# NSagan271/dietgpu_fork

Measured on AMD Instinct MI355X. Metric: encode+decode GB/s (+ratio) on bf16 batch at 1/2/4/8 MI355X vs HBM roofline, higher is better.
Workload: dtype u32; 1 GPU; c2: batch=256 x 1 MiB bf16 N(0,1) per GPU; batch_per_gpu=256, words_per_tensor=524288, prob_bits=10, api=floatCompress + floatDecompress (pointer API, C ABI), parallelism=dp1 (independent shards + RCCL size all-gather)

## Files before the change

### dietgpu_fork_amd/csrc/decode.h

```cpp
#pragma once

#include <type_traits>

#include "archive.h"

namespace dietgpu {

namespace dec {
constexpr int kThreads = 256;
constexpr int kWaves = kThreads / 64;
constexpr uint32_t kRing = 512;
constexpr uint32_t kRefill = 256;
constexpr uint32_t kWPL = kRefill / 64;
constexpr uint32_t kSegSteps = 8;
constexpr uint32_t kSegWords = kSegSteps * 32;
constexpr uint32_t kUnroll = 4;
constexpr uint32_t kChunk = kSegWords / 32;
}

template <int FT>
struct DecCfg {
  static constexpr int S = FloatTraits<FT>::kSegs;
  static constexpr int kBlocksPerWave = 2;
  static constexpr int kBlocksPerWG = dec::kWaves * kBlocksPerWave;
  static constexpr uint32_t kHalfStreams = dec::kWaves * S * 2;
  static constexpr uint32_t kRingBytes = kHalfStreams * dec::kRing * 2;
  static constexpr uint32_t kSegBytes = kHalfStreams * dec::kSegWords * 2;
  __host__ __device__ static constexpr uint32_t lutBytes(int pb) { return S * (8u << pb); }
  __host__ __device__ static constexpr uint32_t ldsBytes(int pb) {
    return lutBytes(pb) + kRingBytes + kSegBytes;
  }
};

struct DStream {
  uint32_t x;
  lp<uint16_t> ring;
  lp<const uint16_t> ringLane;
  int32_t ptr[2];
  int32_t lo[2];
  gp<const uint16_t> data[2];
  u32x2 pf[2];
};

__device__ __forceinline__ u32x2 ld4w(gp<const uint16_t> p, bool vec) {
  if (vec) return *(gp<const u32x2>)p;
  return u32x2{uint32_t(p[0]) | (uint32_t(p[1]) << 16), uint32_t(p[2]) | (uint32_t(p[3]) << 16)};
}

__device__ __forceinline__ void ringPrefetch(DStream& p, int hh, uint32_t lane, bool vec) {
  const int32_t nlo = max(0, p.lo[hh] - int32_t(dec::kRefill));
  if (p.lo[hh] > 0 && int32_t(dec::kWPL * lane) < p.lo[hh] - nlo)
    p.pf[hh] = ld4w(p.data[hh] + nlo + dec::kWPL * lane, vec);
}

__device__ __forceinline__ void ringEnsure(DStream& p, uint32_t lane, bool vec) {
#pragma unroll
  for (int hh = 0; hh < 2; ++hh) {
    if (p.lo[hh] > 0 && p.ptr[hh] - int32_t(32 * dec::kUnroll) < p.lo[hh]) {
      const int32_t nlo = max(0, p.lo[hh] - int32_t(dec::kRefill));
      if (int32_t(dec::kWPL * lane) < p.lo[hh] - nlo)
        *(lp<u32x2>)(p.ring + hh * dec::kRing + ((nlo + dec::kWPL * lane) & (dec::kRing - 1))) = p.pf[hh];
      p.lo[hh] = nlo;
      ringPrefetch(p, hh, lane, vec);
    }
  }
}

template <bool kMask, int NC>
__device__ __forceinline__ void decStepAll(DStream* const (&p)[NC], const bool (&valid)[NC],
                                           lp<const u32x2> const (&lut)[NC], uint32_t mask, int pb,
                                           uint32_t hv, uint32_t (&e0)[NC]) {
  u32x2 e[NC];
#pragma unroll
  for (int c = 0; c < NC; ++c) e[c] = lut[c][p[c]->x & mask];
  __builtin_amdgcn_sched_barrier(0);
  uint32_t xn[NC], v[NC];
  bool rd[NC];
#pragma unroll
  for (int c = 0; c < NC; ++c) {
    DStream& q = *p[c];
    xn[c] = __umul24(e[c].x, q.x >> pb) + e[c].y;
    if (kMask) xn[c] = valid[c] ? xn[c] : q.x;
    rd[c] = kMask ? (valid[c] && xn[c] < kMinState) : (xn[c] < kMinState);
    const uint64_t vote = ballot(rd[c]);
    const int32_t cLo = __popc(uint32_t(vote));
    const int32_t cHi = __popc(uint32_t(vote >> 32));
    const int32_t baseLo = q.ptr[0] - cLo;
    const int32_t diff = q.ptr[1] - q.ptr[0] - cHi;
    q.ptr[0] = baseLo;
    q.ptr[1] -= cHi;
    const uint32_t vbase = uint32_t(baseLo) + (hv & uint32_t(diff));
    const uint32_t idx = __builtin_amdgcn_mbcnt_hi(uint32_t(vote >> 32),
                                                   __builtin_amdgcn_mbcnt_lo(uint32_t(vote), vbase));
    v[c] = q.ringLane[idx & (dec::kRing - 1)];
    e0[c] = e[c].x;
  }
  __builtin_amdgcn_sched_barrier(0);
#pragma unroll
  for (int c = 0; c < NC; ++c)
    p[c]->x = __builtin_amdgcn_perm(xn[c], v[c], rd[c] ? 0x05040100u : 0x07060504u);
}

template <bool kMask, int S>
__device__ __forceinline__ void decSteps(DStream* const (&chains)[S], lp<const u32x2> const (&lut)[S],
                                         uint32_t mask, int pb, uint32_t hv, lp<uint16_t> const (&segLane)[S],
                                         int tr0, int32_t tBot, uint32_t l, uint32_t uw) {
#pragma unroll
  for (int u = int(dec::kUnroll) - 1; u >= 0; --u) {
    const int tr = tr0 + u;
    bool vld[S];
#pragma unroll
    for (int s = 0; s < S; ++s) vld[s] = !kMask || uint32_t(tBot + tr) * 32 + l < uw;
    uint32_t e0[S];
    decStepAll<kMask, S>(chains, vld, lut, mask, pb, hv, e0);
#pragma unroll
    for (int s = 0; s < S; ++s)
      if (vld[s]) segLane[s][tr * 32] = uint16_t(e0[s] >> 16);
  }
}

__device__ __forceinline__ uint32_t upperHalfMask(uint32_t lane) {
  uint32_t hv = lane >= 32 ? ~0u : 0u;
  asm volatile("" : "+v"(hv));
  return hv;
}

__device__ __forceinline__ void bindStream(DStream& d, lp<uint16_t>& segLane, lp<uint16_t> ringAll,
                                           lp<uint16_t> segAll, uint32_t hs, uint32_t hv, uint32_t l) {
  d.ring = ringAll + hs * 2 * dec::kRing;
  d.ringLane = d.ring + (hv & dec::kRing);
  segLane = segAll + hs * 2 * dec::kSegWords + (hv & dec::kSegWords) + l;
}

__device__ __forceinline__ void openHalf(DStream& d, int hh, gp<const uint16_t> data, uint2 e, bool has,
                                         uint32_t lane, bool vecIn) {
  d.ptr[hh] = 0;
  d.lo[hh] = 0;
  d.data[hh] = data;
  d.pf[hh] = u32x2{0, 0};
  if (has) {
    const uint32_t ex = readfirst(e.x), ey = readfirst(e.y);
    const int32_t cw = int32_t(ex & 0xffffu);
    d.ptr[hh] = cw;
    d.data[hh] = data + ey;
    const int32_t lo = cw > int32_t(dec::kRing) ? int32_t(roundUp(uint32_t(cw) - dec::kRing, dec::kWPL)) : 0;
    d.lo[hh] = lo;
#pragma unroll
    for (int q = 0; q < int(dec::kRing / dec::kRefill); ++q) {
      const int32_t a = lo + q * int32_t(dec::kRefill) + int32_t(dec::kWPL * lane);
      if (a < cw) *(lp<u32x2>)(d.ring + hh * dec::kRing + (a & (dec::kRing - 1))) = ld4w(d.data[hh] + a, vecIn);
    }
    ringPrefetch(d, hh, lane, vecIn);
  }
}

__device__ __forceinline__ void setPrioRemaining(uint32_t left, uint32_t total) {
  const uint32_t q = total ? min(3u, (4u * left) / total) : 0u;
  if (q == 3) __builtin_amdgcn_s_setprio(3);
  else if (q == 2) __builtin_amdgcn_s_setprio(2);
  else if (q == 1) __builtin_amdgcn_s_setprio(1);
  else __builtin_amdgcn_s_setprio(0);
}

template <int FT, int ACC = 0>
struct Join {
  static_assert(ACC == 0 || (FT != 0 && (ACC == 1 || (ACC == 2 && (FT == 1 || FT == 2)))),
                "accumulate: float archives only; an fp32 accumulator only for fp16 / bf16");
  using WordT = typename FloatTraits<FT>::WordT;
  using AccT = std::conditional_t<ACC == 2, uint32_t, WordT>;
  static constexpr int kR = FT == 0 ? 1 : (FT <= 2 ? 2 : (FT == 3 ? 6 : 12));
  static constexpr int kW = 2 * int(sizeof(WordT));
  static constexpr int kD = ACC == 0 ? 1 : 2 * int(sizeof(AccT));

  static __device__ __forceinline__ void load(uint32_t (&r)[kR], gp<const uint8_t> raw, uint32_t n,
                                              uint32_t i0) {
    if constexpr (FT == 1 || FT == 2) {
      const uint2 a = ld8(raw + i0);
      r[0] = a.x; r[1] = a.y;
    } else if constexpr (FT == 3) {
      const uint4 a = ld16(raw + 2 * i0);
      const uint2 h = ld8(raw + floatPlane2Offset(FT, n) + i0);
      r[0] = a.x; r[1] = a.y; r[2] = a.z; r[3] = a.w; r[4] = h.x; r[5] = h.y;
    } else if constexpr (FT == 4) {
      const uint4 a = ld16(raw + 4 * i0), b = ld16(raw + 4 * i0 + 16);
      const uint4 h = ld16(raw + floatPlane2Offset(FT, n) + 2 * i0);
      r[0] = a.x; r[1] = a.y; r[2] = a.z; r[3] = a.w;
      r[4] = b.x; r[5] = b.y; r[6] = b.z; r[7] = b.w;
      r[8] = h.x; r[9] = h.y; r[10] = h.z; r[11] = h.w;
    }
  }

  static __device__ __forceinline__ WordT one(uint32_t s0, uint32_t s1, gp<const uint8_t> raw,
                                              uint32_t n, uint32_t i) {
    if constexpr (FT == 0) {
      return WordT(s0);
    } else if constexpr (FT == 1) {
      return WordT((s0 << 8) | raw[i]);
    } else if constexpr (FT == 2) {
      const uint32_t r = raw[i];
      return WordT((s0 << 7) | (r >> 1) | ((r & 1u) << 15));
    } else if constexpr (FT == 3) {
      const uint32_t lo = ((gp<const uint16_t>)raw)[i];
      const uint32_t hb = raw[floatPlane2Offset(FT, n) + i];
      return rotr32((s0 << 24) | (hb << 16) | lo, 1);
    } else {
      const uint64_t lo = ((gp<const uint32_t>)raw)[i];
      const uint64_t hb = ((gp<const uint16_t>)(raw + floatPlane2Offset(FT, n)))[i];
      const uint64_t v = (uint64_t(s0) << 56) | (uint64_t(s1) << 48) | (hb << 32) | lo;
      return (v >> 1) | (v << 63);
    }
  }

  static __device__ __forceinline__ uint32_t pair16(uint32_t sp, uint32_t rw, int odd) {
    return __builtin_amdgcn_perm(sp, rw, odd ? 0x07030502u : 0x07010500u);
  }

  template <bool nt>
  static __device__ __forceinline__ void vec(gp<uint8_t> outB, uint32_t i0, const uint32_t (&s)[4],
                                             const uint32_t (&s1)[4], const uint32_t (&r)[kR]) {
    if constexpr (FT == 0) {
      const uint2 v = make_uint2(__builtin_amdgcn_perm(s[1], s[0], 0x07050301u),
                                 __builtin_amdgcn_perm(s[3], s[2], 0x07050301u));
      if constexpr (nt) st8nt(outB + i0, v);
      else st8(outB + i0, v);
    } else if constexpr (FT == 1 || FT == 2) {
      uint32_t o[4];
#pragma unroll
      for (int k = 0; k < 4; ++k) {
        const uint32_t t = pair16(s[k], r[k >> 1], k & 1);
        o[k] = FT == 1 ? t : (((t >> 1) & 0x7fff7fffu) | ((t << 15) & 0x80008000u));
      }
      if constexpr (nt) st16nt(outB + 2 * i0, make_uint4(o[0], o[1], o[2], o[3]));
      else st16(outB + 2 * i0, make_uint4(o[0], o[1], o[2], o[3]));
    } else if constexpr (FT == 3) {
      uint32_t o[8];
#pragma unroll
      for (int k = 0; k < 4; ++k) {
        const uint32_t h = pair16(s[k], r[4 + (k >> 1)], k & 1);
        const uint32_t w0 = __builtin_amdgcn_perm(h, r[k], 0x05040100u);
        const uint32_t w1 = __builtin_amdgcn_perm(h, r[k], 0x07060302u);
        o[2 * k] = __builtin_amdgcn_alignbit(w0, w0, 1);
        o[2 * k + 1] = __builtin_amdgcn_alignbit(w1, w1, 1);
      }
      gp<uint4> d = (gp<uint4>)(outB + 4 * i0);
      if constexpr (nt) {
        st16nt(d, make_uint4(o[0], o[1], o[2], o[3]));
        st16nt(d + 1, make_uint4(o[4], o[5], o[6], o[7]));
      } else {
        st16(d, make_uint4(o[0], o[1], o[2], o[3]));
        st16(d + 1, make_uint4(o[4], o[5], o[6], o[7]));
      }
    } else {
      gp<uint4> d = (gp<uint4>)(outB + 8 * i0);
#pragma unroll
      for (int k = 0; k < 4; ++k) {
        const uint32_t p = __builtin_amdgcn_perm(s[k], s1[k], 0x07030501u);
        const uint32_t vh0 = __builtin_amdgcn_perm(p, r[8 + k], 0x05040100u);
        const uint32_t vh1 = __builtin_amdgcn_perm(p, r[8 + k], 0x07060302u);
        const uint32_t l0 = r[2 * k], l1 = r[2 * k + 1];
        st16(d + k, make_uint4(__builtin_amdgcn_alignbit(vh0, l0, 1), __builtin_amdgcn_alignbit(l0, vh0, 1),
                               __builtin_amdgcn_alignbit(vh1, l1, 1), __builtin_amdgcn_alignbit(l1, vh1, 1)));
      }
    }
  }

  static __device__ __forceinline__ float widen(uint32_t h) {
    if constexpr (FT == 1) return float(__builtin_bit_cast(_Float16, uint16_t(h)));
    else return __builtin_bit_cast(float, h << 16);
  }
  static __device__ __forceinline__ uint32_t bf16Of(float f) {
    return __builtin_bit_cast(uint16_t, static_cast<__bf16>(f));
  }
  static __device__ __forceinline__ uint32_t f32Sum(uint32_t a, float x) {
    return __builtin_bit_cast(uint32_t, __builtin_bit_cast(float, a) + x);
  }
  static __device__ __forceinline__ uint32_t sumPk16(uint32_t a, uint32_t x) {
    if constexpr (FT == 1) {
      typedef _Float16 h2 __attribute__((ext_vector_type(2)));
      return __builtin_bit_cast(uint32_t, __builtin_bit_cast(h2, a) + __builtin_bit_cast(h2, x));
    } else {
      const float lo = __builtin_bit_cast(float, a << 16) + __builtin_bit_cast(float, x << 16);
      const float hi = __builtin_bit_cast(float, a & 0xffff0000u) + __builtin_bit_cast(float, x & 0xffff0000u);
      return bf16Of(lo) | (bf16Of(hi) << 16);
    }
  }
  static __device__ __forceinline__ AccT sumOne(AccT a, WordT x) {
    if constexpr (ACC == 2) {
      return f32Sum(a, widen(x));
    } else if constexpr (FT == 1) {
      return __builtin_bit_cast(uint16_t, _Float16(__builtin_bit_cast(_Float16, a) + __builtin_bit_cast(_Float16, x)));
    } else if constexpr (FT == 2) {
      return AccT(bf16Of(widen(a) + widen(x)));
    } else if constexpr (FT == 3) {
      return f32Sum(a, __builtin_bit_cast(float, x));
    } else {
      return __builtin_bit_cast(uint64_t, __builtin_bit_cast(double, a) + __builtin_bit_cast(double, x));
    }
  }

  static __device__ __forceinline__ void words(uint32_t (&o)[kW], const uint32_t (&s)[4], const uint32_t (&s1)[4],
                                               const uint32_t (&r)[kR]) {
    if constexpr (FT == 0) {
      o[0] = __builtin_amdgcn_perm(s[1], s[0], 0x07050301u);
      o[1] = __builtin_amdgcn_perm(s[3], s[2], 0x07050301u);
    } else if constexpr (FT == 1 || FT == 2) {
#pragma unroll
      for (int k = 0; k < 4; ++k) {
        const uint32_t t = pair16(s[k], r[k >> 1], k & 1);
        o[k] = FT == 1 ? t : (((t >> 1) & 0x7fff7fffu) | ((t << 15) & 0x80008000u));
      }
    } else if constexpr (FT == 3) {
#pragma unroll
      for (int k = 0; k < 4; ++k) {
        const uint32_t h = pair16(s[k], r[4 + (k >> 1)], k & 1);
        const uint32_t w0 = __builtin_amdgcn_perm(h, r[k], 0x05040100u);
        const uint32_t w1 = __builtin_amdgcn_perm(h, r[k], 0x07060302u);
        o[2 * k] = __builtin_amdgcn_alignbit(w0, w0, 1);
        o[2 * k + 1] = __builtin_amdgcn_alignbit(w1, w1, 1);
      }
    } else {
#pragma unroll
      for (int k = 0; k < 4; ++k) {
        const uint32_t p = __builtin_amdgcn_perm(s[k], s1[k], 0x07030501u);
        const uint32_t vh0 = __builtin_amdgcn_perm(p, r[8 + k], 0x05040100u);
        const uint32_t vh1 = __builtin_amdgcn_perm(p, r[8 + k], 0x07060302u);
        const uint32_t l0 = r[2 * k], l1 = r[2 * k + 1];
        o[4 * k] = __builtin_amdgcn_alignbit(vh0, l0, 1);
        o[4 * k + 1] = __builtin_amdgcn_alignbit(l0, vh0, 1);
        o[4 * k + 2] = __builtin_amdgcn_alignbit(vh1, l1, 1);
        o[4 * k + 3] = __builtin_amdgcn_alignbit(l1, vh1, 1);
      }
    }
  }

  static __device__ __forceinline__ void loadAcc(uint32_t (&d)[kD], gp<const uint8_t> accB, uint32_t i0) {
    gp<const u32x4> p = (gp<const u32x4>)(accB + uint64_t(sizeof(AccT)) * i0);
#pragma unroll
    for (int j = 0; j < kD / 4; ++j) {
      const u32x4 v = p[j];
      d[4 * j] = v.x; d[4 * j + 1] = v.y; d[4 * j + 2] = v.z; d[4 * j + 3] = v.w;
    }
  }

  static __device__ __forceinline__ void vecAcc(gp<uint8_t> accB, uint32_t i0, const uint32_t (&s)[4],
                                                const uint32_t (&s1)[4], const uint32_t (&r)[kR],
                                                const uint32_t (&d)[kD]) {
    gp<u32x4> p = (gp<u32x4>)(accB + uint64_t(sizeof(AccT)) * i0);
    uint32_t o[kW], t[kD];
    if constexpr (FT == 4) {
      loadAcc(t, accB, i0);
      words(o, s, s1, r);
#pragma unroll
      for (int k = 0; k < 8; ++k) {
        const uint64_t sum = sumOne(uint64_t(t[2 * k]) | (uint64_t(t[2 * k + 1]) << 32),
                                    uint64_t(o[2 * k]) | (uint64_t(o[2 * k + 1]) << 32));
        t[2 * k] = uint32_t(sum);
        t[2 * k + 1] = uint32_t(sum >> 32);
      }
    } else {
      words(o, s, s1, r);
      if constexpr (ACC == 2) {
#pragma unroll
        for (int k = 0; k < 4; ++k) {
          t[2 * k] = f32Sum(d[2 * k], widen(o[k]));
          t[2 * k + 1] = f32Sum(d[2 * k + 1], widen(o[k] >> 16));
        }
      } else if constexpr (FT == 3) {
#pragma unroll
        for (int k = 0; k < 8; ++k) t[k] = f32Sum(d[k], __builtin_bit_cast(float, o[k]));
      } else {
#pragma unroll
        for (int k = 0; k < 4; ++k) t[k] = sumPk16(d[k], o[k]);
      }
    }
#pragma unroll
    for (int j = 0; j < kD / 4; ++j) p[j] = u32x4{t[4 * j], t[4 * j + 1], t[4 * j + 2], t[4 * j + 3]};
  }
};

template <int S>
__device__ __forceinline__ void loadChunkSyms(lp<const uint16_t> q0, lp<const uint16_t> q1, uint32_t (&sv)[4],
                                              uint32_t (&sv1)[4]) {
  const u32x4 a0 = *(lp<const u32x4>)q0;
  sv[0] = a0.x; sv[1] = a0.y; sv[2] = a0.z; sv[3] = a0.w;
  if constexpr (S == 2) {
    const u32x4 b0 = *(lp<const u32x4>)q1;
    sv1[0] = b0.x; sv1[1] = b0.y; sv1[2] = b0.z; sv1[3] = b0.w;
  } else {
#pragma unroll
    for (int k = 0; k < 4; ++k) sv1[k] = 0;
  }
}

__device__ __forceinline__ bool clipChunk(uint32_t i0, uint32_t cnt, uint32_t rlo, uint32_t rhi, uint32_t& k0,
                                          uint32_t& k1) {
  k0 = i0 < rlo ? min(cnt, rlo - i0) : 0u;
  k1 = rhi > i0 ? min(cnt, rhi - i0) : 0u;
  return k0 < k1;
}

template <class J>
__device__ __forceinline__ void joinWords(gp<typename J::WordT> o, lp<const uint16_t> q0, lp<const uint16_t> q1,
                                          gp<const uint8_t> raw, uint32_t n, uint32_t i0, uint32_t k0, uint32_t k1) {
  for (uint32_t k = k0; k < k1; ++k) o[i0 + k] = J::one(q0[k] >> 8, q1[k] >> 8, raw, n, i0 + k);
}

template <int FT>
__device__ __forceinline__ uint32_t openArchive(gp<const uint8_t> base, int pb, bool& ok,
                                                gp<const uint8_t> (&arch)[DecCfg<FT>::S]) {
  constexpr int S = DecCfg<FT>::S;
  gp<const uint32_t> fh = (gp<const uint32_t>)base;
  uint32_t n;
  if constexpr (FT == 0) {
    n = fh[kAnsSize];
    ok = fh[kAnsMagic] == kANSMagicVersion;
  } else {
    n = fh[kFloatSize];
    ok = fh[kFloatMagic] == kFloatMagicVersion && (fh[kFloatType] & kTypeMask) == uint32_t(FT);
  }
  arch[0] = ansArchiveOf<FT>(base, n);
  if constexpr (S == 2) arch[S - 1] = arch[0] + fh[kFloatSecondAns];
#pragma unroll
  for (int s = 0; s < S; ++s) {
    gp<const uint32_t> ah = (gp<const uint32_t>)arch[s];
    ok = ok && ah[kAnsMagic] == kANSMagicVersion && (ah[kAnsPrecision] & kTypeMask) == uint32_t(pb) &&
         ah[kAnsSize] == n;
  }
  return n;
}

__device__ __forceinline__ void buildLut64(gp<const uint16_t> pdfIn, lp<u32x2> lut, int pb,
                                           uint32_t* scratch) {
  static_assert(dec::kThreads == kNumSymbols, "one symbol per thread");
  uint32_t* cdfS = scratch;
  uint32_t* pdfS = scratch + kNumSymbols;
  uint32_t* red = scratch + 2 * kNumSymbols;
  const uint32_t tid = threadIdx.x;
  const uint32_t p = pdfIn[tid];
  const uint32_t c = blockExclusiveScan<dec::kThreads>(p, red, nullptr);
  pdfS[tid] = p;
  cdfS[tid] = c;
  __syncthreads();
  constexpr int kG = 4;
  const uint32_t total = 1u << pb;
#pragma unroll 1
  for (uint32_t g0 = tid; g0 < total; g0 += kG * dec::kThreads) {
    uint32_t s[kG], cs[kG];
#pragma unroll
    for (int j = 0; j < kG; ++j) s[j] = 0, cs[j] = 0;
#pragma unroll
    for (uint32_t bit = kNumSymbols / 2; bit; bit >>= 1) {
#pragma unroll
      for (int j = 0; j < kG; ++j) {
        const uint32_t cv = cdfS[s[j] + bit];
        const bool up = cv <= g0 + j * dec::kThreads;
        s[j] = up ? s[j] + bit : s[j];
        cs[j] = up ? cv : cs[j];
      }
    }
#pragma unroll
    for (int j = 0; j < kG; ++j) {
      const uint32_t slot = g0 + j * dec::kThreads;
      if (slot < total) lut[slot] = u32x2{pdfS[s[j]] | (s[j] << 24), slot - cs[j]};
    }
  }
}

template <int FT, bool NT, bool BAL, bool RNG = false, int ACC = 0>
__global__ __launch_bounds__(dec::kThreads) __attribute__((amdgpu_num_sgpr(80), amdgpu_waves_per_eu(4))) void k_decode(const InlineTable,
                                                          BatchDesc in, BatchDesc out,
                                                          uint32_t batchOffset, int pb,
                                                          uint32_t chunksPerWG,
                                                          uint8_t* __restrict__ outSuccess,
                                                          uint32_t* __restrict__ outSize) {
  using Cfg = DecCfg<FT>;
  using WordT = typename FloatTraits<FT>::WordT;
  using J = Join<FT, ACC>;
  using AccT = typename J::AccT;
  constexpr int S = Cfg::S, R = J::kR, D = J::kD;
  static_assert(!(ACC && (RNG || NT || BAL)), "accumulate: whole elements, plain stores, no priorities");
  constexpr bool kAccAhead = ACC != 0 && FT != 4;
  extern __shared__ __attribute__((aligned(16))) uint8_t smem[];
  lp<uint8_t> L = (lp<uint8_t>)smem;
  const uint32_t lutBytes = Cfg::lutBytes(pb);
  lp<uint16_t> ringAll = (lp<uint16_t>)(L + lutBytes);
  lp<uint16_t> segAll = (lp<uint16_t>)(L + lutBytes + Cfg::kRingBytes);

  const uint32_t b = batchOffset + blockIdx.y;
  const uint32_t tid = threadIdx.x;
  gp<const uint8_t> base = startOf(in, b);

  gp<const uint8_t> arch[S];
  bool ok;
  const uint32_t n = openArchive<FT>(base, pb, ok, arch);
  uint32_t rlo = 0, rhi = 0;
  bool success;
  if constexpr (RNG) {
    static_assert(!BAL, "range decode: no priorities");
    rlo = in.size(b);
    const uint32_t count = out.size(b);
    success = ok && rlo <= n && count <= n - rlo;
    rhi = success ? rlo + count : rlo;
    if (blockIdx.x == 0 && tid == 0) {
      if (outSuccess) outSuccess[b] = success ? 1 : 0;
      if (outSize) outSize[b] = success ? count : 0u;
    }
  } else {
    success = ok && out.size(b) >= n;
    if (blockIdx.x == 0 && tid == 0) {
      if (outSuccess) outSuccess[b] = success ? 1 : 0;
      if (outSize) outSize[b] = ok ? n : 0u;
    }
  }
  const uint32_t nBlocks = divUp(n, kBlockSize);
  const uint32_t blkFirst = RNG ? rlo / kBlockSize : 0u;
  const uint32_t blkEnd = RNG ? divUp(rhi, kBlockSize) : nBlocks;
  if constexpr (RNG) {
    if (!success || rhi == rlo || blkFirst + blockIdx.x * chunksPerWG * Cfg::kBlocksPerWG >= blkEnd) return;
  } else {
    if (!success || blockIdx.x * chunksPerWG * Cfg::kBlocksPerWG >= nBlocks) return;
  }

  const uint32_t w = readfirst(tid >> 6), lane = tid & 63, l = lane & 31;
  const uint32_t hv = upperHalfMask(lane);

  const bool vecIn = (reinterpret_cast<uintptr_t>(base) & 15) == 0;
  gp<uint8_t> outB = startOf(out, b);
  if constexpr (RNG)
    outB = (gp<uint8_t>)(reinterpret_cast<uintptr_t>(outB) - uint64_t(rlo) * sizeof(WordT));
  const bool vecOut = (reinterpret_cast<uintptr_t>(outB) & 15) == 0;
  auto wholeInRange = [&](uint32_t i0) __attribute__((always_inline)) {
    return !RNG || (i0 >= rlo && i0 + dec::kChunk <= rhi);
  };
  gp<const uint8_t> raw = rawSectionOf(base);
  const uint32_t mask = (1u << pb) - 1;
  lp<const u32x2> lut[S];
#pragma unroll
  for (int s = 0; s < S; ++s) lut[s] = (lp<const u32x2>)(L + s * (lutBytes / S));

  const bool vecIO = vecIn && vecOut;
  uint32_t x0[S];
  uint2 bwE[S][2];
  uint32_t rvA[R], rvB[R];
  uint32_t dvA[D], dvB[D];
  auto issue = [&](uint32_t blk0) __attribute__((always_inline)) {
    const uint32_t off = dec::kChunk * l;
    const uint32_t bkMine = blk0 + (lane >> 5);
    const uint32_t uwMin = min(blockSymbols(blk0 + 1, blkEnd, n), blockSymbols(blk0, blkEnd, n));
    const uint32_t iTop = bkMine * kBlockSize + (kBlockSize / 32 / dec::kSegSteps - 1) * dec::kSegWords + off;
    if (FT != 0 && vecIO && uwMin == kBlockSize && wholeInRange(iTop)) {
      J::load(rvA, raw, n, iTop);
      if constexpr (kAccAhead) J::loadAcc(dvA, outB, iTop);
    }
#pragma unroll
    for (int s = 0; s < S; ++s) {
      const AnsSections arc(arch[s], nBlocks);
      x0[s] = bkMine < blkEnd ? ((gp<const uint32_t>)(arc.states + uint64_t(kStateBytesPerBlock) * bkMine))[l]
                              : kMinState;
#pragma unroll
      for (int hh = 0; hh < 2; ++hh) {
        const uint32_t bk = blk0 + hh;
        bwE[s][hh] = bk < blkEnd ? ld8(arc.bwords + bk) : make_uint2(0, 0);
      }
    }
  };
  {
    const uint32_t blk00 = blkFirst + blockIdx.x * chunksPerWG * Cfg::kBlocksPerWG + w * Cfg::kBlocksPerWave;
    if (blk00 < blkEnd) issue(blk00);
  }
#pragma unroll
  for (int s = 0; s < S; ++s) {
    buildLut64((gp<const uint16_t>)(arch[s] + kANSHeaderBytes),
               (lp<u32x2>)(L + s * (lutBytes / S)), pb, (uint32_t*)segAll);
    __syncthreads();
  }

  for (uint32_t pass = 0; pass < chunksPerWG; ++pass) {
    const uint32_t blk0 =
        blkFirst + (blockIdx.x * chunksPerWG + pass) * Cfg::kBlocksPerWG + w * Cfg::kBlocksPerWave;
    if (blk0 >= blkEnd) break;
    if (pass > 0) issue(blk0);

    uint32_t uwH[2];
    DStream st[S];
    lp<uint16_t> segLane[S];
#pragma unroll
    for (int hh = 0; hh < 2; ++hh) uwH[hh] = blockSymbols(blk0 + hh, blkEnd, n);
    int32_t gMin = 0;
    if constexpr (RNG) {
      if (blk0 == blkFirst && blk0 + 1 >= blkEnd) gMin = int32_t((rlo - blkFirst * kBlockSize) / dec::kSegWords);
    }
    const uint32_t T = max(divUp(uwH[0], 32), divUp(uwH[1], 32));
    const uint32_t nFull = min(uwH[0], uwH[1]) / dec::kSegWords;
    const int32_t nSeg = int32_t(divUp(T, dec::kSegSteps));
    const uint32_t off = dec::kChunk * l;

    const bool rawEarly = FT != 0 && vecIO && nSeg > 0 && uint32_t(nSeg - 1) < nFull;
#pragma unroll
    for (int s = 0; s < S; ++s) {
      gp<const uint16_t> data = AnsSections(arch[s], nBlocks).words;
      bindStream(st[s], segLane[s], ringAll, segAll, w * S + s, hv, l);
#pragma unroll
      for (int hh = 0; hh < 2; ++hh) openHalf(st[s], hh, data, bwE[s][hh], blk0 + hh < blkEnd, lane, vecIn);
      st[s].x = x0[s];
    }

    DStream* chains[S];
#pragma unroll
    for (int s = 0; s < S; ++s) chains[s] = &st[s];

    auto run = [&](auto vecTag) {
      constexpr bool kVec = decltype(vecTag)::value;
      auto loadRaw = [&](int32_t g, bool fullSeg, uint32_t (&rv)[R], uint32_t (&dv)[D]) {
        const uint32_t segW0 = uint32_t(g) * dec::kSegWords;
        const uint32_t uw = lane >= 32 ? uwH[1] : uwH[0];
        const uint32_t bk = blk0 + (lane >> 5);
        if (FT != 0 && kVec && (fullSeg || segW0 + off + dec::kChunk <= uw) &&
            wholeInRange(bk * kBlockSize + segW0 + off)) {
          J::load(rv, raw, n, bk * kBlockSize + segW0 + off);
          if constexpr (kAccAhead) J::loadAcc(dv, outB, bk * kBlockSize + segW0 + off);
        }
      };
      auto join = [&](int32_t g, bool fullSeg, const uint32_t (&rv)[R], const uint32_t (&dv)[D]) {
        const uint32_t segW0 = uint32_t(g) * dec::kSegWords;
        const uint32_t uw = lane >= 32 ? uwH[1] : uwH[0];
        const uint32_t bk = blk0 + (lane >> 5);
        if (!fullSeg && segW0 + off >= uw) return;
        const uint32_t cnt = fullSeg ? dec::kChunk : min(dec::kChunk, uw - segW0 - off);
        const uint32_t i0 = bk * kBlockSize + segW0 + off;
        uint32_t k0 = 0, k1 = cnt;
        if constexpr (RNG) {
          if (!clipChunk(i0, cnt, rlo, rhi, k0, k1)) return;
        }
        lp<const uint16_t> q0 = segLane[0] - l + off;
        lp<const uint16_t> q1 = segLane[S - 1] - l + off;
        if (kVec && cnt == dec::kChunk && wholeInRange(i0)) {
          uint32_t sv[4], sv1[4];
          loadChunkSyms<S>(q0, q1, sv, sv1);
          if constexpr (ACC) J::vecAcc(outB, i0, sv, sv1, rv, dv);
          else J::template vec<NT>(outB, i0, sv, sv1, rv);
        } else if constexpr (ACC) {
          gp<AccT> a = (gp<AccT>)outB + uint64_t(i0);
          for (uint32_t k = k0; k < k1; ++k) a[k] = J::sumOne(a[k], J::one(q0[k] >> 8, q1[k] >> 8, raw, n, i0 + k));
        } else {
          joinWords<J>((gp<WordT>)outB, q0, q1, raw, n, i0, k0, k1);
        }
      };

      if (nSeg > 0 && !(kVec && rawEarly)) loadRaw(nSeg - 1, uint32_t(nSeg - 1) < nFull, rvA, dvA);
      const int32_t gStop = RNG ? max(int32_t(nFull), gMin) : int32_t(nFull);
      for (int32_t g = nSeg - 1; g >= gStop; --g) {
        const int32_t tBot = g * int32_t(dec::kSegSteps);
#pragma unroll
        for (int grp = int(dec::kSegSteps / dec::kUnroll) - 1; grp >= 0; --grp) {
#pragma unroll
          for (int s = 0; s < S; ++s) ringEnsure(st[s], lane, kVec);
          decSteps<true, S>(chains, lut, mask, pb, hv, segLane, grp * int(dec::kUnroll), tBot, l,
                            lane >= 32 ? uwH[1] : uwH[0]);
        }
        __builtin_amdgcn_wave_barrier();
        join(g, false, rvA, dvA);
        __builtin_amdgcn_wave_barrier();
        if (g > gMin) loadRaw(g - 1, uint32_t(g - 1) < nFull, rvA, dvA);
      }
      auto fullSeg = [&](int32_t g, const uint32_t (&cur)[R], uint32_t (&nxt)[R], const uint32_t (&dcur)[D],
                         uint32_t (&dnxt)[D]) {
        if constexpr (BAL)
          setPrioRemaining((chunksPerWG - 1 - pass) * uint32_t(nSeg) + uint32_t(g), chunksPerWG * uint32_t(nSeg));
        if (g > 0) loadRaw(g - 1, true, nxt, dnxt);
#pragma unroll
        for (int grp = int(dec::kSegSteps / dec::kUnroll) - 1; grp >= 0; --grp) {
#pragma unroll
          for (int s = 0; s < S; ++s) ringEnsure(st[s], lane, kVec);
          decSteps<false, S>(chains, lut, mask, pb, hv, segLane, grp * int(dec::kUnroll), 0, l, 0u);
        }
        __builtin_amdgcn_wave_barrier();
        join(g, true, cur, dcur);
        __builtin_amdgcn_wave_barrier();
      };
      int32_t g = min(nSeg, int32_t(nFull)) - 1;
      for (; g >= 1; g -= 2) {
        fullSeg(g, rvA, rvB, dvA, dvB);
        fullSeg(g - 1, rvB, rvA, dvB, dvA);
      }
      if (g == 0) fullSeg(0, rvA, rvB, dvA, dvB);
    };
    if (vecIn && vecOut)
      run(std::true_type{});
    else
      run(std::false_type{});
    __builtin_amdgcn_wave_barrier();
  }
}

}
```

Measured before the change: 1307 GB/s.

## Streamline decode ring refill bookkeeping, hoist ensure per segment, cache priority thresholds

```diff
diff --git a/dietgpu_fork_amd/csrc/decode.h b/dietgpu_fork_amd/csrc/decode.h
--- a/dietgpu_fork_amd/csrc/decode.h
+++ b/dietgpu_fork_amd/csrc/decode.h
@@ -36,33 +36,44 @@
   uint32_t x;
   lp<uint16_t> ring;
   lp<const uint16_t> ringLane;
-  int32_t ptr[2];
-  int32_t lo[2];
+  int32_t ptr;
+  int32_t gap;
+  int32_t need[2];
   gp<const uint16_t> data[2];
   u32x2 pf[2];
 };
 
+namespace dec {
+constexpr int32_t kNoRefill = -(1 << 30);
+}
+
 __device__ __forceinline__ u32x2 ld4w(gp<const uint16_t> p, bool vec) {
   if (vec) return *(gp<const u32x2>)p;
   return u32x2{uint32_t(p[0]) | (uint32_t(p[1]) << 16), uint32_t(p[2]) | (uint32_t(p[3]) << 16)};
 }
 
 __device__ __forceinline__ void ringPrefetch(DStream& p, int hh, uint32_t lane, bool vec) {
-  const int32_t nlo = max(0, p.lo[hh] - int32_t(dec::kRefill));
-  if (p.lo[hh] > 0 && int32_t(dec::kWPL * lane) < p.lo[hh] - nlo)
+  const int32_t lo = p.need[hh] - int32_t(dec::kRefill);
+  const int32_t nlo = max(0, lo - int32_t(dec::kRefill));
+  if (p.need[hh] > 0 && int32_t(dec::kWPL * lane) < lo - nlo)
     p.pf[hh] = ld4w(p.data[hh] + nlo + dec::kWPL * lane, vec);
 }
 
+__device__ __forceinline__ void ringRefill(DStream& p, int hh, uint32_t lane, bool vec) {
+  const int32_t lo = p.need[hh] - int32_t(dec::kRefill);
+  const int32_t nlo = max(0, lo - int32_t(dec::kRefill));
+  if (int32_t(dec::kWPL * lane) < lo - nlo)
+    *(lp<u32x2>)(p.ring + hh * dec::kRing + ((nlo + dec::kWPL * lane) & (dec::kRing - 1))) = p.pf[hh];
+  p.need[hh] = nlo > 0 ? nlo + int32_t(dec::kRefill) : dec::kNoRefill;
+  ringPrefetch(p, hh, lane, vec);
+}
+
 __device__ __forceinline__ void ringEnsure(DStream& p, uint32_t lane, bool vec) {
-#pragma unroll
-  for (int hh = 0; hh < 2; ++hh) {
-    if (p.lo[hh] > 0 && p.ptr[hh] - int32_t(32 * dec::kUnroll) < p.lo[hh]) {
-      const int32_t nlo = max(0, p.lo[hh] - int32_t(dec::kRefill));
-      if (int32_t(dec::kWPL * lane) < p.lo[hh] - nlo)
-        *(lp<u32x2>)(p.ring + hh * dec::kRing + ((nlo + dec::kWPL * lane) & (dec::kRing - 1))) = p.pf[hh];
-      p.lo[hh] = nlo;
-      ringPrefetch(p, hh, lane, vec);
-    }
+  static_assert(dec::kSegSteps * 32 <= dec::kRefill && 2 * dec::kRefill == dec::kRing, "a segment's words per refill");
+  const int32_t ptr1 = p.ptr + p.gap;
+  if (((p.ptr - p.need[0]) | (ptr1 - p.need[1])) < 0) {
+    if (p.ptr < p.need[0]) ringRefill(p, 0, lane, vec);
+    if (ptr1 < p.need[1]) ringRefill(p, 1, lane, vec);
   }
 }
 
@@ -81,15 +92,15 @@
     DStream& q = *p[c];
     xn[c] = __umul24(e[c].x, q.x >> pb) + e[c].y;
     if (kMask) xn[c] = valid[c] ? xn[c] : q.x;
-    rd[c] = kMask ? (valid[c] && xn[c] < kMinState) : (xn[c] < kMinState);
-    const uint64_t vote = ballot(rd[c]);
+    const bool lt = xn[c] < kMinState;
+    rd[c] = kMask ? (valid[c] && lt) : lt;
+    const uint64_t vote = kMask ? (ballot(lt) & ballot(valid[c])) : ballot(lt);
     const int32_t cLo = __popc(uint32_t(vote));
     const int32_t cHi = __popc(uint32_t(vote >> 32));
-    const int32_t baseLo = q.ptr[0] - cLo;
-    const int32_t diff = q.ptr[1] - q.ptr[0] - cHi;
-    q.ptr[0] = baseLo;
-    q.ptr[1] -= cHi;
-    const uint32_t vbase = uint32_t(baseLo) + (hv & uint32_t(diff));
+    const int32_t up = q.gap - cHi;
+    q.ptr -= cLo;
+    q.gap = up + cLo;
+    const uint32_t vbase = uint32_t(q.ptr) + (hv & uint32_t(up));
     const uint32_t idx = __builtin_amdgcn_mbcnt_hi(uint32_t(vote >> 32),
                                                    __builtin_amdgcn_mbcnt_lo(uint32_t(vote), vbase));
     v[c] = q.ringLane[idx & (dec::kRing - 1)];
@@ -134,17 +145,17 @@
 
 __device__ __forceinline__ void openHalf(DStream& d, int hh, gp<const uint16_t> data, uint2 e, bool has,
                                          uint32_t lane, bool vecIn) {
-  d.ptr[hh] = 0;
-  d.lo[hh] = 0;
+  int32_t top = 0;
+  d.need[hh] = dec::kNoRefill;
   d.data[hh] = data;
   d.pf[hh] = u32x2{0, 0};
   if (has) {
     const uint32_t ex = readfirst(e.x), ey = readfirst(e.y);
     const int32_t cw = int32_t(ex & 0xffffu);
-    d.ptr[hh] = cw;
+    top = cw;
     d.data[hh] = data + ey;
     const int32_t lo = cw > int32_t(dec::kRing) ? int32_t(roundUp(uint32_t(cw) - dec::kRing, dec::kWPL)) : 0;
-    d.lo[hh] = lo;
+    if (lo > 0) d.need[hh] = lo + int32_t(dec::kRefill);
 #pragma unroll
     for (int q = 0; q < int(dec::kRing / dec::kRefill); ++q) {
       const int32_t a = lo + q * int32_t(dec::kRefill) + int32_t(dec::kWPL * lane);
@@ -152,14 +163,33 @@
     }
     ringPrefetch(d, hh, lane, vecIn);
   }
-}
-
-__device__ __forceinline__ void setPrioRemaining(uint32_t left, uint32_t total) {
-  const uint32_t q = total ? min(3u, (4u * left) / total) : 0u;
-  if (q == 3) __builtin_amdgcn_s_setprio(3);
-  else if (q == 2) __builtin_amdgcn_s_setprio(2);
-  else if (q == 1) __builtin_amdgcn_s_setprio(1);
-  else __builtin_amdgcn_s_setprio(0);
+  if (hh == 0) {
+    d.ptr = top;
+    d.gap = -top;
+  } else {
+    d.gap += top;
+  }
+}
+
+__device__ __forceinline__ int32_t setPrioRemaining(int32_t g, uint32_t nSeg, uint32_t passesLeft, uint32_t passes) {
+  const uint32_t total = passes * nSeg;
+  const int32_t base = int32_t(passesLeft * nSeg);
+  const int32_t at3 = int32_t((3 * total + 3) >> 2) - base, at2 = int32_t((2 * total + 3) >> 2) - base,
+                at1 = int32_t((total + 3) >> 2) - base;
+  if (g >= at3) {
+    __builtin_amdgcn_s_setprio(3);
+    return at3;
+  }
+  if (g >= at2) {
+    __builtin_amdgcn_s_setprio(2);
+    return at2;
+  }
+  if (g >= at1) {
+    __builtin_amdgcn_s_setprio(1);
+    return at1;
+  }
+  __builtin_amdgcn_s_setprio(0);
+  return INT32_MIN;
 }
 
 template <int FT, int ACC = 0>
@@ -652,28 +682,28 @@
       for (int32_t g = nSeg - 1; g >= gStop; --g) {
         const int32_t tBot = g * int32_t(dec::kSegSteps);
 #pragma unroll
-        for (int grp = int(dec::kSegSteps / dec::kUnroll) - 1; grp >= 0; --grp) {
-#pragma unroll
-          for (int s = 0; s < S; ++s) ringEnsure(st[s], lane, kVec);
+        for (int s = 0; s < S; ++s) ringEnsure(st[s], lane, kVec);
+#pragma unroll
+        for (int grp = int(dec::kSegSteps / dec::kUnroll) - 1; grp >= 0; --grp)
           decSteps<true, S>(chains, lut, mask, pb, hv, segLane, grp * int(dec::kUnroll), tBot, l,
                             lane >= 32 ? uwH[1] : uwH[0]);
-        }
         __builtin_amdgcn_wave_barrier();
         join(g, false, rvA, dvA);
         __builtin_amdgcn_wave_barrier();
         if (g > gMin) loadRaw(g - 1, uint32_t(g - 1) < nFull, rvA, dvA);
       }
+      int32_t prioBelow = INT32_MAX;
       auto fullSeg = [&](int32_t g, const uint32_t (&cur)[R], uint32_t (&nxt)[R], const uint32_t (&dcur)[D],
                          uint32_t (&dnxt)[D]) {
-        if constexpr (BAL)
-          setPrioRemaining((chunksPerWG - 1 - pass) * uint32_t(nSeg) + uint32_t(g), chunksPerWG * uint32_t(nSeg));
+        if constexpr (BAL) {
+          if (g < prioBelow) prioBelow = setPrioRemaining(g, uint32_t(nSeg), chunksPerWG - 1 - pass, chunksPerWG);
+        }
         if (g > 0) loadRaw(g - 1, true, nxt, dnxt);
 #pragma unroll
-        for (int grp = int(dec::kSegSteps / dec::kUnroll) - 1; grp >= 0; --grp) {
-#pragma unroll
-          for (int s = 0; s < S; ++s) ringEnsure(st[s], lane, kVec);
+        for (int s = 0; s < S; ++s) ringEnsure(st[s], lane, kVec);
+#pragma unroll
+        for (int grp = int(dec::kSegSteps / dec::kUnroll) - 1; grp >= 0; --grp)
           decSteps<false, S>(chains, lut, mask, pb, hv, segLane, grp * int(dec::kUnroll), 0, l, 0u);
-        }
         __builtin_amdgcn_wave_barrier();
         join(g, true, cur, dcur);
         __builtin_amdgcn_wave_barrier();
```

After: 1275 GB/s. -2.5%, worse.
